# MorphIQ-Labs/VectorWave

Hardware: AMD Instinct MI355X
Metric: Msamples/sec MODWT fwd+inv db4 L=6, batch 4096×4096 fp64 @ 1/2/4/8 GPU (higher is better)
Workload: dtype f64

## Files before the change

include/vectorwave_amd.h:

```cpp
#ifndef VECTORWAVE_AMD_H
#define VECTORWAVE_AMD_H

#include <stdint.h>

#ifdef __cplusplus
extern "C" {
#endif

#define VW_API __attribute__((visibility("default")))

typedef struct vw_ctx vw_ctx;
typedef struct vw_stream vw_stream;
typedef int vw_status;

enum {
    VW_OK = 0,
    VW_ERR_NULL = 1,
    VW_ERR_EMPTY = 2,
    VW_ERR_NONFINITE = 3,
    VW_ERR_LEVEL = 4,
    VW_ERR_TOO_LARGE = 5,
    VW_ERR_BOUNDARY = 6,
    VW_ERR_ARG = 7,
    VW_ERR_DEVICE = 8,
// ... 178 lines not shown

VW_API vw_status vw_stream_create(vw_ctx *ctx, const double *lo, const double *hi, int L,
                                  int boundary, int levels, vw_stream **out);
VW_API vw_status vw_stream_destroy(vw_stream *s);
VW_API vw_status vw_stream_process_f64(vw_stream *s, const double *block, int64_t B, int64_t n,
                                       unsigned flags, double *details, double *approx);
VW_API vw_status vw_stream_flush_f64(vw_stream *s, int64_t tail_len, unsigned flags,
                                     double *details, double *approx);
VW_API int64_t vw_stream_history_length(vw_stream *s, int level);
VW_API int64_t vw_stream_batch(vw_stream *s);

typedef struct vw_graph vw_graph;
VW_API vw_status vw_capture_begin(vw_ctx *ctx);
VW_API vw_status vw_capture_end(vw_ctx *ctx, vw_graph **out);
VW_API vw_status vw_graph_launch(vw_graph *graph, int64_t count);
VW_API vw_status vw_graph_destroy(vw_graph *graph);
VW_API vw_status vw_graph_stats(vw_graph *graph, int *kernel_nodes, int *fused_pairs);

VW_API vw_status vw_modwt_roundtrip_f64(vw_ctx *ctx, const double *x, int64_t B, int64_t N, int64_t ldx,
                                        const double *lo, const double *hi, const double *rlo, const double *rhi,
                                        int L, int wavelet_id, int boundary, int J, unsigned flags, double *details,
                                        double *approx, double *y);
VW_API vw_status vw_roundtrip_occupancy(vw_ctx *ctx, int64_t N, int L, int J, unsigned flags, int *per_cu);

typedef struct vw_pipeline vw_pipeline;
VW_API vw_status vw_pipeline_create(vw_ctx *fwd_ctx, vw_ctx *inv_ctx, int elem_bytes, int sets, void *const *x,
                                    void *const *details, void *const *approx, void *const *y, int64_t B,
                                    int64_t N, const double *lo, const double *hi, int L, int wavelet_id,
                                    int boundary, int J, unsigned flags, vw_pipeline **out);
VW_API vw_status vw_pipeline_run(vw_pipeline *p, int64_t steps);
VW_API vw_status vw_pipeline_join(vw_pipeline *p);
VW_API int64_t vw_pipeline_last_set(vw_pipeline *p);
VW_API vw_status vw_pipeline_destroy(vw_pipeline *p);

VW_API vw_status vw_fill_uniform_f64(vw_ctx *ctx, double *x, int64_t count, uint64_t seed, int64_t offset);
VW_API vw_status vw_fill_uniform_f32(vw_ctx *ctx, float *x, int64_t count, uint64_t seed, int64_t offset);
VW_API vw_status vw_device_alloc(vw_ctx *ctx, int64_t bytes, void **out);
VW_API vw_status vw_device_free(vw_ctx *ctx, void *p);
VW_API vw_status vw_memcpy(vw_ctx *ctx, void *dst, const void *src, int64_t bytes, int kind );

VW_API vw_status vw_ctx_enable_timing(vw_ctx *ctx, int enable);
VW_API vw_status vw_ctx_kernel_time(vw_ctx *ctx, const char *family, double *total_ms, int64_t *launches);
VW_API vw_status vw_ctx_reset_timing(vw_ctx *ctx);
VW_API vw_status vw_ctx_kernel_spans(vw_ctx *ctx, const char *family, void *ref_event, int64_t max,
                                     double *start_ms, double *end_ms, int64_t *count);

// ... 5 lines not shown
```

vectorwave_amd/_native.py:

```python
from __future__ import annotations

import ctypes
import os
from ctypes import POINTER, c_char_p, c_double, c_float, c_int, c_int64, c_uint, c_uint64, c_void_p

_HERE = os.path.dirname(os.path.abspath(__file__))
LIB_PATH = os.environ.get("VW_LIB_PATH", os.path.join(_HERE, "libvectorwave_amd.so"))

FLAG_CORE_LEVELS = 1 << 0
FLAG_VALIDATE = 1 << 1
FLAG_FFT_SWITCH = 1 << 2
FLAG_FMA = 1 << 3
FLAG_HOST_MEMORY = 1 << 4
FLAG_SYNC = 1 << 5
FLAG_BATCH_SYM_INVERSE = 1 << 6
FLAG_BATCH_HAAR = 1 << 7
FLAG_REF_NONFINITE = 1 << 8
FLAG_TREE_SUMS = 1 << 9

PERIODIC, SYMMETRIC, ZERO_PADDING = 0, 1, 2

CWT_ZERO, CWT_REFLECT, CWT_SYMMETRIC, CWT_PERIODIC, CWT_WRAP_ZERO = 0, 1, 2, 3, 4


# ... 85 lines not shown
    "vw_stream_history_length": (c_int64, [c_void_p, c_int]),
    "vw_stream_batch": (c_int64, [c_void_p]),
    "vw_fill_uniform_f64": (c_int, [c_void_p, c_void_p, c_int64, c_uint64, c_int64]),
    "vw_fill_uniform_f32": (c_int, [c_void_p, c_void_p, c_int64, c_uint64, c_int64]),
    "vw_device_alloc": (c_int, [c_void_p, c_int64, POINTER(c_void_p)]),
    "vw_device_free": (c_int, [c_void_p, c_void_p]),
    "vw_memcpy": (c_int, [c_void_p, c_void_p, c_void_p, c_int64, c_int]),
    "vw_ctx_enable_timing": (c_int, [c_void_p, c_int]),
    "vw_ctx_kernel_time": (c_int, [c_void_p, c_char_p, POINTER(c_double), POINTER(c_int64)]),
    "vw_ctx_reset_timing": (c_int, [c_void_p]),
    "vw_ctx_kernel_spans": (c_int, [c_void_p, c_char_p, c_void_p, c_int64, POINTER(c_double), POINTER(c_double),
                                    POINTER(c_int64)]),
    "vw_median_f64": (c_int, [c_void_p, c_void_p, c_int64, c_int64, c_void_p, c_uint, c_void_p]),
    "vw_stddev_f64": (c_int, [c_void_p, c_void_p, c_int64, c_uint, c_void_p]),
    "vw_window_gather_abs_f64": (c_int, [c_void_p, c_void_p, c_void_p, c_int64, c_void_p, c_int64, c_int64]),
    "vw_capture_begin": (c_int, [c_void_p]),
    "vw_capture_end": (c_int, [c_void_p, POINTER(c_void_p)]),
    "vw_graph_launch": (c_int, [c_void_p, c_int64]),
    "vw_graph_destroy": (c_int, [c_void_p]),
    "vw_graph_stats": (c_int, [c_void_p, POINTER(c_int), POINTER(c_int)]),
    "vw_modwt_roundtrip_f64": (c_int, [c_void_p, c_void_p, c_int64, c_int64, c_int64, _dp, _dp, _dp, _dp, c_int, c_int,
                                       c_int, c_int, c_uint, c_void_p, c_void_p, c_void_p]),
    "vw_roundtrip_occupancy": (c_int, [c_void_p, c_int64, c_int, c_int, c_uint, POINTER(c_int)]),
    "vw_pipeline_create": (c_int, [c_void_p, c_void_p, c_int, c_int, c_void_p, c_void_p, c_void_p, c_void_p, c_int64,
                                   c_int64, _dp, _dp, c_int, c_int, c_int, c_int, c_uint, POINTER(c_void_p)]),
    "vw_pipeline_run": (c_int, [c_void_p, c_int64]),
    "vw_pipeline_join": (c_int, [c_void_p]),
    "vw_pipeline_last_set": (c_int64, [c_void_p]),
    "vw_pipeline_destroy": (c_int, [c_void_p]),
}

_lib = None


def load() -> ctypes.CDLL:
    global _lib
    if _lib is not None:
        return _lib
    if not os.path.exists(LIB_PATH):
        raise ImportError(
            f"vectorwave_amd native library not found at {LIB_PATH}; build it with "
            f"`python -c 'import __graft_entry__ as g; g.build()'` (make -C vectorwave_amd/csrc)")
    lib = ctypes.CDLL(LIB_PATH)
    for name, (res, args) in SIGNATURES.items():
        fn = getattr(lib, name)
        fn.restype = res
# ... 18 lines not shown
```

vectorwave_amd/csrc/vw_capi.cpp:

```cpp
#include "../../include/vectorwave_amd.h"
#include "vw_internal.h"
#include "vw_deep.h"
#include "vw_plan.h"

#include <algorithm>
#include <cmath>
#include <cstdarg>
#include <cstdio>
#include <cstring>
#include <map>
#include <mutex>
#include <set>
#include <string>
#include <thread>
#include <vector>

using namespace vw;

static thread_local std::string t_err;
static thread_local int64_t t_err_index = -1;
static thread_local int64_t t_signal_base = 0;

static vw_status fail(vw_status code, const char* fmt, ...) {
  char buf[512];
// ... 856 lines not shown
static bool capture_tail(hipStream_t st, hipGraphNode_t* node) {
  hipStreamCaptureStatus status;
  unsigned long long id = 0;
  hipGraph_t g = nullptr;
  const hipGraphNode_t* deps = nullptr;
  size_t ndeps = 0;
  if (hipStreamGetCaptureInfo_v2(st, &status, &id, &g, &deps, &ndeps) != hipSuccess) {
    (void)hipGetLastError();
    return false;
  }
  if (status != hipStreamCaptureStatusActive || ndeps != 1 || !deps) return false;
  *node = deps[0];
  return true;
}

static bool pair_forward_shape(const FwdPlan<double>& p) {
  return p.fused && p.kernel == kFwdPersist && p.args.level_ct && p.nv == 4 && p.args.taps <= kPairMaxTaps;
}

static void pair_after_forward(vw_ctx* c, const FwdCall<double>& k, const FwdPlan<double>& p, const FwdArgs<double>& a) {
  c->pair.valid = false;
  if (!c->tune.pair_fuse || !pair_forward_shape(p)) return;
  if (!c->capturing) {
    if (pair_prepare(a.taps, p.fma, p.threads, p.lds, nullptr) != hipSuccess) (void)hipGetLastError();
    return;
  }
  if (c->timing || p.ref_nf || p.validate) return;
  hipGraphNode_t node = nullptr;
  hipGraphNodeType ty;
  if (!capture_tail(c->stream, &node)) return;
  if (hipGraphNodeGetType(node, &ty) != hipSuccess || ty != hipGraphNodeTypeKernel) {
    (void)hipGetLastError();
    return;
  }
  c->pair.node = node;
  c->pair.call = k;
  c->pair.call.lo = c->pair.call.hi = nullptr;
  c->pair.plan = p;
  c->pair.args = a;
  c->pair.valid = true;
}
static void pair_after_forward(vw_ctx* c, const FwdCall<float>&, const FwdPlan<float>&, const FwdArgs<float>&) {
  c->pair.valid = false;
}

static void pair_args(const FwdArgs<double>& f, const InvCall<double>& k, const InvPlan<double>& p, PairArgs<double>* a) {
  a->f = f;
  a->y = k.y;
  double lo[kMaxTaps], hi[kMaxTaps];
  copy_bank(lo, hi, k, p.args.taps, p.args.taps_hi);
  for (int i = 0; i < kPairMaxTaps; ++i) { a->ilo[i] = lo[i]; a->ihi[i] = hi[i]; }
  for (int j = 0; j < kMaxLevels; ++j) { a->hr[j] = p.args.lv[j].hr; a->own[j] = p.args.lv[j].own; }
}

static bool try_pair_fuse(vw_ctx* c, const InvCall<double>& k, const InvPlan<double>& p) {
  const bool pending = c->pair.valid;
  c->pair.valid = false;
  if (!pending || !c->capturing || c->timing || !c->tune.pair_fuse) return false;
  hipGraphNode_t tail = nullptr;
  if (!capture_tail(c->stream, &tail) || tail != c->pair.node) return false;
  if (!pair_fusable(c->pair.call, c->pair.plan, k, p)) return false;
  const FwdPlan<double>& fp = c->pair.plan;
  PairLaunch l;
  if (!pair_launch_shape(fp.args.taps, fp.fma, fp.threads, fp.lds, k.B, c->cus, &l)) return false;
  PairArgs<double> a;
  pair_args(c->pair.args, k, p, &a);
  void* params[] = {&a};
  hipKernelNodeParams np;
  memset(&np, 0, sizeof(np));
  np.func = const_cast<void*>(l.func);
  np.gridDim = dim3(l.grid);
  np.blockDim = dim3(l.threads);
  np.sharedMemBytes = l.lds;
  np.kernelParams = params;
  if (hipGraphKernelNodeSetParams(c->pair.node, &np) != hipSuccess) {
    (void)hipGetLastError();
    return false;
  }
  ++c->fused_pairs;
  return true;
}
static bool try_pair_fuse(vw_ctx* c, const InvCall<float>&, const InvPlan<float>&) {
  c->pair.valid = false;
  return false;
}

template <typename T>
// ... 344 lines not shown
}

extern "C" vw_status vw_modwt_roundtrip_f64(vw_ctx* c, const double* x, int64_t B, int64_t N, int64_t ldx,
                                            const double* lo, const double* hi, const double* rlo, const double* rhi,
                                            int L, int wid, int boundary, int J, unsigned flags, double* details,
                                            double* approx, double* y) {
  if (c && x && details && approx && y && lo && hi && rlo && rhi && !(flags & VW_FLAG_HOST_MEMORY) && B > 0 && N > 0 &&
      ldx >= N && L >= 1 && L <= kPairMaxTaps && J >= 1 && J <= kMaxLevels && boundary == VW_PERIODIC) {
    std::lock_guard<std::recursive_mutex> g(c->mu);
    hipSetDevice(c->device);
    FwdCall<double> fk;
    fk.x = x; fk.B = B; fk.N = N; fk.ldx = ldx; fk.lo = lo; fk.hi = hi; fk.L = L; fk.boundary = boundary; fk.J = J;
    fk.flags = flags; fk.details = details; fk.approx = approx; fk.cus = c->cus;
    InvCall<double> ik;
    ik.details = details; ik.approx = approx; ik.B = B; ik.N = N; ik.lo = rlo; ik.hi = rhi; ik.L = L; ik.wid = wid;
    ik.boundary = boundary; ik.J = J; ik.flags = flags; ik.y = y; ik.cus = c->cus;
    FwdPlan<double> fp;
    InvPlan<double> ip;
    if (c->tune.pair_fuse && check_levels(N, L, J, flags) == VW_OK && capture_guard(c, flags) == VW_OK) {
      plan_forward(c->tune, fk, &fp);
      plan_inverse(c->tune, ik, &ip);
      PairLaunch l;
      if (pair_fusable(fk, fp, ik, ip) &&
          (c->capturing || pair_prepare(fp.args.taps, fp.fma, fp.threads, fp.lds, nullptr) == hipSuccess) &&
          pair_launch_shape(fp.args.taps, fp.fma, fp.threads, fp.lds, B, c->cus, &l)) {
        FwdArgs<double> f = fp.args;
        f.x = x; f.details = details; f.approx = approx;
        f.bad = c->bad;
        copy_bank(f.lo, f.hi, fk, f.taps, f.taps_hi);
        PairArgs<double> a;
        pair_args(f, ik, ip, &a);
        {
          LaunchTimer lt(c, "roundtrip");
          hipError_t e = launch_roundtrip(a, l, c->stream);
          if (e != hipSuccess) return fail(VW_ERR_DEVICE, "round-trip launch failed: %s", hipGetErrorString(e));
        }
        if (flags & VW_FLAG_SYNC) VW_HIP(hipStreamSynchronize(c->stream));
        return ok();
      }
      (void)hipGetLastError();
    }
  }
  VW_TRY(modwt_forward<double>(c, x, B, N, ldx, lo, hi, L, wid, boundary, J, flags, details, approx));
  return modwt_inverse<double>(c, details, approx, B, N, rlo, rhi, L, wid, boundary, J, ~0u, 0, flags, y);
}

extern "C" vw_status vw_roundtrip_occupancy(vw_ctx* c, int64_t N, int L, int J, unsigned flags, int* per_cu) {
  if (!c || !per_cu) return fail(VW_ERR_NULL, "null argument");
  *per_cu = 0;
  if (N <= 0 || N > (1LL << 30) || L < 1 || L > kPairMaxTaps || J < 1 || J > kMaxLevels) return ok();
  std::lock_guard<std::recursive_mutex> g(c->mu);
  if (c->capturing) return fail(VW_ERR_STATE, "occupancy queries cannot be captured");
  hipSetDevice(c->device);
  double* const aligned = reinterpret_cast<double*>(uintptr_t(4096));
  static const double taps[kPairMaxTaps] = {0};
  FwdCall<double> fk;
  fk.x = aligned; fk.details = aligned; fk.approx = aligned;
  fk.B = 4LL * c->cus; fk.N = N; fk.ldx = N; fk.lo = taps; fk.hi = taps; fk.L = L; fk.J = J;
  fk.flags = flags & VW_FLAG_FMA; fk.cus = c->cus;
  FwdPlan<double> fp;
  plan_forward(c->tune, fk, &fp);
  if (fp.error != VW_OK || !pair_forward_shape(fp)) return ok();
  if (pair_prepare(fp.args.taps, fp.fma, fp.threads, fp.lds, per_cu) != hipSuccess) {
    (void)hipGetLastError();
    *per_cu = 0;
  }
  return ok();
}

static int bank_hi(int Llo, int Lhi) { return Lhi == Llo ? 0 : Lhi; }
static vw_status bank_arg(int Lhi) {
  if (Lhi < 1 || Lhi > kMaxTaps) return fail(VW_ERR_ARG, "filter length %d unsupported (1..%d)", Lhi, kMaxTaps);
  return VW_OK;
}
extern "C" vw_status vw_modwt_forward_bi_f64(vw_ctx* c, const double* x, int64_t B, int64_t N, int64_t ldx,
                                             const double* lo, int Llo, const double* hi, int Lhi, int wid,
                                             int boundary, int J, unsigned flags, double* details, double* approx) {
  VW_TRY(bank_arg(Lhi));
  return modwt_forward<double>(c, x, B, N, ldx, lo, hi, Llo, wid, boundary, J, flags, details, approx, bank_hi(Llo, Lhi));
}
extern "C" vw_status vw_modwt_forward_bi_f32(vw_ctx* c, const float* x, int64_t B, int64_t N, int64_t ldx,
                                             const double* lo, int Llo, const double* hi, int Lhi, int wid,
                                             int boundary, int J, unsigned flags, float* details, float* approx) {
  VW_TRY(bank_arg(Lhi));
  return modwt_forward<float>(c, x, B, N, ldx, lo, hi, Llo, wid, boundary, J, flags, details, approx, bank_hi(Llo, Lhi));
}
extern "C" vw_status vw_modwt_inverse_bi_f64(vw_ctx* c, const double* details, const double* approx, int64_t B,
                                             int64_t N, const double* lo, int Llo, const double* hi, int Lhi, int wid,
                                             int boundary, int J, unsigned detail_mask, int approx_zero,
                                             unsigned flags, double* y) {
// ... 1350 lines not shown
```

vectorwave_amd/csrc/vw_internal.h:

```cpp
#pragma once
#include <hip/hip_runtime.h>
#include <atomic>
#include <cstdint>
#include "vw_taps.h"

namespace vw {

constexpr int kMaxTaps = 64;
constexpr int kMaxLevels = 24;
constexpr int kNV = 8;
constexpr int kMaxThreads = 1024;
constexpr int kLdsBytes = 160 * 1024;
constexpr int kSweepMinS = 16;
constexpr int kSweepChunk = 128;

enum HaloMode : int {
  kHaloPeriodic = 0,
  kHaloZero = 1,
  kHaloSymmetric = 2,
  kHaloFftPad = 3,
  kHaloHistory = 4
};

struct LevelDesc {
// ... 58 lines not shown
  int unrolled;
  int level_ct;
  int full;
  int plain;
  int waves;
  int db;
  int blk;
  int approx_zero;
  int rev;
  const T* thr;
  long long thr_ld;
  int soft;
  int taps;
  int taps_hi;
  int tap_lds;
  int blk_tight;
  int* nf_flag;
  T lo[kMaxTaps];
  T hi[kMaxTaps];
  LevelDesc lv[kMaxLevels];
};

constexpr int kPairMaxTaps = 8;
template <typename T>
struct PairArgs {
  FwdArgs<T> f;
  T* y;
  T ilo[kPairMaxTaps];
  T ihi[kPairMaxTaps];
  int hr[kMaxLevels];
  int own[kMaxLevels];
};

template <typename T>
struct LevelArgs {
  const T* src_a;
  long long lda;
  const T* src_d;
  const T* src_d2;
  const T* thr2;
  int use_d2;
  const T* src_d3;
  const T* thr3;
  int use_d3;
  T* out_a;
  T* out_d;
// ... 235 lines not shown
  if (lds_bytes <= 64 * 1024) return hipSuccess;
  int dev = 0;
  if (hipGetDevice(&dev) != hipSuccess || dev < 0) dev = 0;
  std::atomic<int>* f = dev < kMaxDevices ? &once->limit[dev] : nullptr;
  if (f && f->load(std::memory_order_acquire) >= lds_bytes) return hipSuccess;
  if (want < lds_bytes) want = lds_bytes;
  hipError_t e = hipFuncSetAttribute(reinterpret_cast<const void*>(k), hipFuncAttributeMaxDynamicSharedMemorySize, want);
  if (e != hipSuccess) return e;
  if (f) f->store(want, std::memory_order_release);
  return hipSuccess;
}

template <typename T>
hipError_t launch_forward_fused(const FwdArgs<T>& a, int threads, int lds_bytes, bool fma, int nv, hipStream_t st);
template <typename T>
hipError_t launch_forward_persist(const FwdArgs<T>& a, int threads, int lds_bytes, bool fma, int nv, hipStream_t st);
template <typename T>
hipError_t launch_forward_blk(const FwdArgs<T>& a, int threads, int lds_bytes, bool fma, int nv, hipStream_t st);
template <typename T>
hipError_t launch_inverse_fused(const InvArgs<T>& a, int threads, int lds_bytes, bool fma, int nv, hipStream_t st);
struct PairLaunch {
  const void* func;
  unsigned grid, threads, lds;
};
hipError_t pair_prepare(int taps, bool fma, int threads, int lds_bytes, int* per_cu);
bool pair_launch_shape(int taps, bool fma, int threads, int lds_bytes, long long B, int cus, PairLaunch* out);
hipError_t launch_roundtrip(const PairArgs<double>& a, const PairLaunch& l, hipStream_t st);
template <typename T>
hipError_t launch_forward_level(const LevelArgs<T>& a, int lds_bytes, bool fma, hipStream_t st);
template <typename T>
hipError_t launch_inverse_level(const LevelArgs<T>& a, int lds_bytes, bool fma, hipStream_t st);
template <typename T>
hipError_t launch_forward_sweep(const LevelArgs<T>& a, bool fma, hipStream_t st);
template <typename T>
hipError_t launch_inverse_sweep(const LevelArgs<T>& a, bool fma, hipStream_t st);
template <typename T>
hipError_t launch_inverse_sweepg(const LevelArgs<T>& a, int levels, int ka, int R, bool fma, hipStream_t st);
template <typename T>
hipError_t launch_forward_multi(const MultiArgs<T>& a, int lds_bytes, bool fma, hipStream_t st);

template <typename T>
hipError_t launch_inverse_multi(const MultiArgs<T>& a, int lds_bytes, bool fma, hipStream_t st);
template <typename T>
hipError_t launch_history_update(const T* level_in, long long ld_in, const T* old_hist, T* new_hist,
                                 long long B, int n, int hist_len, hipStream_t st);

hipError_t launch_level_threshold(const double* coeffs, long long level_stride, const double* sigma,
                                  const DenoiseConsts& k, long long B, int levels, double* thr, hipStream_t st);
hipError_t launch_noise_sigma(const double* coeffs, long long ld, long long B, int N, double scale_c,
// ... 32 lines not shown
```

vectorwave_amd/csrc/vw_pair.hip:

```cpp
#include "vw_device.h"

#include <algorithm>
#include <mutex>

namespace vw {

#ifndef VW_PAIR_STORE_AUX
#define VW_PAIR_STORE_AUX 16
#endif

template <typename P>
__device__ __forceinline__ const P* reread(const P* p) {
  int z = 0;
  asm volatile("" : "+s"(z));
  return p + z;
}

template <typename T, int L, bool FMA>
__global__ void __attribute__((amdgpu_flat_work_group_size(1, 512), amdgpu_waves_per_eu(4)))
k_roundtrip(const PairArgs<T> q) {
  constexpr int V = VT<T>::V;
  constexpr int NV = 4;
  const FwdArgs<T>& p = q.f;
  extern __shared__ __attribute__((aligned(16))) unsigned char smem[];
  const int N = p.N;
  const int nvec = N / V;
  const long long G = gridDim.x;
  const size_t plane = (size_t)p.B * (size_t)(unsigned)p.N;
  const unsigned slab = blockDim.x * 16u;
  long long b = blockIdx.x;
  if (b >= p.B) return;
  int cur = 0;
  dma_row<T>(reinterpret_cast<T*>(smem) + p.hlpad, p.x + b * p.ldx, nvec, p.dma_nt != 0);
  wait_vmem();
  for (;;) {
    const FwdArgs<T>& p0 = *reread(&q.f);
    T* X = reinterpret_cast<T*>(smem) + (cur ? p0.region1 : 0) + p0.hlpad;
    T* Y = reinterpret_cast<T*>(smem) + (cur ? 0 : p0.region1) + p0.hlpad;
    lds_barrier();
    fill_halo(X, p0.N, p0.lv[0].hl, p0.lv[0].hr, p0.lv[0].mode, p0.npow2, (const T*)nullptr, 0);
    const long long bn = b + G;
    const size_t row = (size_t)b * (size_t)(unsigned)N;
    const int J = p0.J;
    T acc[NV][V];
    T dlast[NV][V];
    T dreg[NV][V];
    for (int j = 1; j <= J; ++j) {
      const FwdArgs<T>& pj = *reread(&q.f);
      const LevelDesc lv = pj.lv[j - 1];
      lds_barrier();
      if (j == pj.J && bn < pj.B) dma_row<T>(Y, pj.x + bn * pj.ldx, nvec, pj.dma_nt != 0);
      T* dout = pj.details + (size_t)(j - 1) * plane + row;
      T* aout = (j == pj.J) ? pj.approx + row : nullptr;
      fwd_level<T, L, FMA, NV, false, false, true, L, VW_PAIR_STORE_AUX>(p, X, nvec, lv, dout, aout, true, 0ull, acc,
                                                                         nullptr, dlast);
      if (j < pj.J) {
        regs_to_level<T, L, NV, true>(Y, acc, nvec, pj.N, pj.lv[j], pj.npow2, (const T*)nullptr);
        T* t = X; X = Y; Y = t;
      }
    }
    const PairArgs<T>& qi = *reread(&q);
    T* const R = X - qi.f.hlpad;
    lds_barrier();
    plain_to_level<T, NV>(R, acc, slab, qi.f.N, qi.hr[qi.f.J - 1], qi.own[qi.f.J - 1]);
    for (int j = J; j >= 1; --j) {
      const PairArgs<T>& qj = *reread(&q);
      const int s = qj.f.lv[j - 1].s;
      lds_barrier();
      zero_regs<T, NV>(acc);
      plain_row<T, L, FMA, NV, 4>(R, slab, s, qj.ilo, acc);
      lds_barrier();
      if (j < qj.f.J) {
        wait_vmem();
        plain_to_level<T, NV>(R, dreg, slab, qj.f.N, qj.hr[j - 1], qj.own[j - 1]);
      } else {
        plain_to_level<T, NV>(R, dlast, slab, qj.f.N, qj.hr[j - 1], qj.own[j - 1]);
      }
      if (j > 1) {
        if (j == qj.f.J) {
          if (bn < qj.f.B) wait_vmcnt<3 * NV>();
          else wait_vmcnt<2 * NV>();
        }
        plain_load_row<T, NV>(dreg, qj.f.details + (size_t)(j - 2) * plane + row, slab);
      }
      lds_barrier();
      plain_row<T, L, FMA, NV, 4>(R, slab, s, reread(q.ihi), acc);
      if (j > 1) {
        lds_barrier();
        plain_to_level<T, NV>(R, acc, slab, qj.f.N, qj.hr[j - 2], qj.own[j - 2]);
      }
    }
    plain_store_row<T, NV>(q.y + row, acc, slab);
    if (bn >= p.B) break;
    wait_vmcnt<3 * NV>();
    cur = (cur + J) & 1;
    b = bn;
  }
}

struct PairKernel {
  static constexpr int kShapes = 16;
  const void* func = nullptr;
  LdsOnce lds;
  std::mutex mu;
  struct Shape { int threads = -1, lds = -1, per_cu = 0; } shapes[kShapes];
  int next = 0;
  int find(int threads, int lds_bytes) {
    for (const Shape& sh : shapes)
      if (sh.threads == threads && sh.lds == lds_bytes) return sh.per_cu;
    return 0;
  }
};

template <int L, bool FMA>
static PairKernel* pair_kernel_of() {
  static PairKernel k;
  k.func = reinterpret_cast<const void*>(&k_roundtrip<double, L, FMA>);
  return &k;
}

static PairKernel* pair_kernel(int taps, bool fma) {
  switch (taps) {
#define VW_CASE(n) \
    case n:        \
      if constexpr (n <= kPairMaxTaps) return fma ? pair_kernel_of<n, true>() : pair_kernel_of<n, false>(); \
      break;
    VW_TAP_LIST(VW_CASE)
#undef VW_CASE
    default: break;
  }
  return nullptr;
}

static bool lds_ready(PairKernel* k, int lds) {
  if (lds <= 64 * 1024) return true;
  int dev = 0;
  if (hipGetDevice(&dev) != hipSuccess || dev < 0 || dev >= kMaxDevices) return false;
  return k->lds.limit[dev].load(std::memory_order_acquire) >= lds;
}

hipError_t pair_prepare(int taps, bool fma, int threads, int lds, int* per_cu) {
  PairKernel* k = pair_kernel(taps, fma);
  if (!k) return hipErrorNotSupported;
  hipError_t e = set_lds(k->func, lds, &k->lds);
  if (e != hipSuccess) return e;
  std::lock_guard<std::mutex> g(k->mu);
  int n = k->find(threads, lds);
  if (!n) {
    if ((e = hipOccupancyMaxActiveBlocksPerMultiprocessor(&n, k->func, threads, lds)) != hipSuccess) return e;
    if (n < 1) return hipErrorInvalidConfiguration;
    PairKernel::Shape& sh = k->shapes[k->next];
    k->next = (k->next + 1) % PairKernel::kShapes;
    sh.threads = threads; sh.lds = lds; sh.per_cu = n;
  }
  if (per_cu) *per_cu = n;
  return hipSuccess;
}

bool pair_launch_shape(int taps, bool fma, int threads, int lds, long long B, int cus, PairLaunch* out) {
  PairKernel* k = pair_kernel(taps, fma);
  if (!k || !lds_ready(k, lds)) return false;
  int n;
  {
    std::lock_guard<std::mutex> g(k->mu);
    n = k->find(threads, lds);
  }
  if (n < 1) return false;
  out->func = k->func;
  out->grid = (unsigned)std::min<long long>(B, (long long)n * cus);
  out->threads = (unsigned)threads;
  out->lds = (unsigned)lds;
  return true;
}

hipError_t launch_roundtrip(const PairArgs<double>& a, const PairLaunch& l, hipStream_t st) {
  void* params[] = {const_cast<PairArgs<double>*>(&a)};
  return hipLaunchKernel(l.func, dim3(l.grid), dim3(l.threads), params, l.lds, st);
}

}
```

vectorwave_amd/csrc/vw_plan.cpp:

```cpp
#include "vw_plan.h"

#include <algorithm>
#include <cstdio>
#include <cstdlib>
#include <cstring>
#include <type_traits>

namespace vw {

struct TuningKey {
  const char* name;
  void (*set)(Tuning& t, const Tuning& d, int v);
};
#define VW_KEY(name, stmt) {name, [](Tuning& t, const Tuning& d, int v) { (void)d; stmt; }}
static const TuningKey kTuningTable[] = {
    VW_KEY("VW_NV", t.nv = v < 0 ? d.nv : v <= 4 ? 4 : 8),
    VW_KEY("VW_FWD_PERSIST", t.fwd_persist = v < 0 ? d.fwd_persist : v != 0),
    VW_KEY("VW_FWD_BUF", t.fwd_buf = v < 0 ? d.fwd_buf : v),
    VW_KEY("VW_FORCE_TILED", t.force_tiled = v > 0),
    VW_KEY("VW_FWD_REV", t.fwd_rev = v < 0 ? 0 : v),
    VW_KEY("VW_INV_REV", t.inv_rev = v < 0 ? 0 : v),
    VW_KEY("VW_FWD_TILE", t.fwd_tile = v < 0 ? 0 : v),
    VW_KEY("VW_MULTI", t.multi = v < 0 ? d.multi : v != 0),
    VW_KEY("VW_MULTI_DIV", t.multi_div = v <= 0 ? d.multi_div : v),
// ... 13 lines not shown
    VW_KEY("VW_DEEP", t.deep = v < 0 ? d.deep : v != 0; t.deep_inv = v < 0 ? d.deep_inv : v != 0),
    VW_KEY("VW_DEEP_INV", t.deep_inv = v < 0 ? d.deep_inv : v != 0),
    VW_KEY("VW_DEEP_LDS", t.deep_lds = v <= 0 ? d.deep_lds : v),
    VW_KEY("VW_DEEP_WAVES", t.deep_waves = v <= 0 ? d.deep_waves : v),
    VW_KEY("VW_DEEP_PF_FWD", t.deep_pf_fwd = v <= 0 ? d.deep_pf_fwd : std::min(v, 16)),
    VW_KEY("VW_DEEP_PF_INV", t.deep_pf_inv = v <= 0 ? d.deep_pf_inv : std::min(v, 16)),
    VW_KEY("VW_SWEEP2", t.sweep2 = v < 0 ? d.sweep2 : v),
    VW_KEY("VW_SWEEP2_KA", t.sweep2_ka = v == 16 ? 16 : v == 8 ? 8 : d.sweep2_ka),
    VW_KEY("VW_SWEEP2_UC", t.sweep2_uc = v >= 32 ? v : d.sweep2_uc),
    VW_KEY("VW_SWEEP2_R", t.sweep2_r = v == 32 ? 32 : 0),
    VW_KEY("VW_SWEEP2_MINB", t.sweep2_minb = v < 0 ? d.sweep2_minb : v),
    VW_KEY("VW_BLK_FWD8", t.blk_fwd8 = v < 0 ? d.blk_fwd8 : v),
    VW_KEY("VW_DMA_NT", t.dma_nt = v < 0 ? d.dma_nt : v),
    VW_KEY("VW_MULTI_NI", t.multi_ni = v < 0 ? d.multi_ni : v == 4 ? 4 : 8),
    VW_KEY("VW_MFMA", t.mfma = v < 0 ? d.mfma : v),
    VW_KEY("VW_REF_GRID", t.ref_grid = v < 0 ? d.ref_grid : v),
    VW_KEY("VW_LEVEL_CT", t.level_ct = v < 0 ? d.level_ct : v != 0),
    VW_KEY("VW_ENERGY_FUSED", t.energy_fused = v < 0 ? d.energy_fused : v),
    VW_KEY("VW_MRA_FUSED", t.mra_fused = v < 0 ? d.mra_fused : v >= 2 ? 2 : v),
    VW_KEY("VW_BI", t.bi = v < 0 ? d.bi : v & 7),
    VW_KEY("VW_BI_LISTED", t.bi_listed = v < 0 ? d.bi_listed : v != 0),
    VW_KEY("VW_INV_WAVES", t.inv_waves = v == 6 || v == 8 ? v : d.inv_waves),
    VW_KEY("VW_PAIR_FUSE", t.pair_fuse = v < 0 ? d.pair_fuse : v != 0),
};
#undef VW_KEY

bool set_tuning(Tuning& t, const char* key, int v) {
  const Tuning d;
  for (const TuningKey& k : kTuningTable)
    if (!strcmp(k.name, key)) { k.set(t, d, v); return true; }
  return false;
}

Tuning read_tuning() {
  Tuning t;
  const Tuning d;
  for (const TuningKey& k : kTuningTable) {
    const char* e = getenv(k.name);
    if (e) k.set(t, d, *e == '\0' ? 1 : atoi(e));
  }
  return t;
}


int max_levels(int64_t N, int L) {
  if (L <= 0 || N <= L) return 0;
// ... 964 lines not shown
  const unsigned off = VW_FLAG_VALIDATE | VW_FLAG_REF_NONFINITE | VW_FLAG_HOST_MEMORY;
  if ((fc.flags | ic.flags) & off) return false;
  if (fc.hist || fp.validate || fp.ref_nf || ip.ref_nf || fp.snapshot) return false;
  if (fp.kernel != kFwdPersist || !fp.args.level_ct || fp.nv != 4 || fp.args.region1 <= 0) return false;
  if (L > kPairMaxTaps || !has_unrolled_taps(L) || fp.args.taps != L || fp.args.taps_hi != L) return false;
  const InvArgs<T>& ia = ip.args;
  if (ip.threads != fp.threads || ip.nv != 4 || ia.taps != L || ia.taps_hi != L) return false;
  if (!ia.plain && !(ip.kernel == kInvDb && plain_class(ic, ip, ip.nv))) return false;
  for (int j = 0; j < J; ++j)
    if (ia.lv[j].s != fp.args.lv[j].s || N + ia.lv[j].hr > fp.args.region1) return false;
  if (fp.lds < 2 * fp.args.region1 * (int)sizeof(T)) return false;
  const size_t row = (size_t)N * sizeof(T), plane = (size_t)B * row;
  const size_t x_bytes = ((size_t)(B - 1) * (size_t)fc.ldx + (size_t)N) * sizeof(T);
  if (ranges_overlap(ic.y, plane, fc.x, x_bytes) || ranges_overlap(ic.y, plane, fc.details, (size_t)J * plane) ||
      ranges_overlap(ic.y, plane, fc.approx, plane))
    return false;
  return true;
}
template bool pair_fusable<float>(const FwdCall<float>&, const FwdPlan<float>&, const InvCall<float>&,
                                  const InvPlan<float>&);
template bool pair_fusable<double>(const FwdCall<double>&, const FwdPlan<double>&, const InvCall<double>&,
                                   const InvPlan<double>&);

template void plan_forward<float>(const Tuning&, const FwdCall<float>&, FwdPlan<float>*);
template void plan_forward<double>(const Tuning&, const FwdCall<double>&, FwdPlan<double>*);
template void plan_inverse<float>(const Tuning&, const InvCall<float>&, InvPlan<float>*);
template void plan_inverse<double>(const Tuning&, const InvCall<double>&, InvPlan<double>*);

}
```

vectorwave_amd/csrc/vw_plan.h:

```cpp
#pragma once
#include "../../include/vectorwave_amd.h"
#include "vw_internal.h"
#include "vw_deep.h"

#include <vector>

namespace vw {

struct Tuning {
  int nv = 4;
  bool fwd_persist = true;
  int fwd_buf = 0;
  bool force_tiled = false;
  int fwd_rev = 0, inv_rev = 0;
  int dma_nt = -1;
  int fwd_tile = 0;
  bool multi = true;
  int multi_div = 4;
  int multi_tile = 0;
  int inv_buf = 0;
  int inv_tile = 0;
  int multi_rblk = 1;
  int multi_pf = 1;
  int multi_pad = 1;
// ... 5 lines not shown
  int blk = 10;
  bool deep = true;
  bool deep_inv = false;
  int deep_lds = 80;
  int deep_waves = 4;
  int deep_pf_fwd = 1;
  int deep_pf_inv = 1;
  int fwd_nv = 0;
  int inv_nv = 0;
  int sweep2 = 3;
  int sweep2_ka = 8;
  int sweep2_uc = 2048;
  int sweep2_r = 0;
  int sweep2_minb = 64;
  int blk_fwd8 = 1;
  int ref_grid = 0;
  int level_ct = 1;
  int mfma = 0;
  int energy_fused = 1;
  int bi = 3;
  int inv_waves = 6;
  int mra_fused = 1;
  int pair_fuse = 1;
  int bi_listed = 1;
};

bool set_tuning(Tuning& t, const char* key, int v);
Tuning read_tuning();

int max_levels(int64_t N, int L);
int64_t upsampled_length(int L, int level);
int ref_mode(int boundary);

template <typename T>
struct FwdCall {
  const T* x = nullptr;
  int64_t B = 0, N = 0, ldx = 0;
  const double* lo = nullptr;
  const double* hi = nullptr;
  int L = 0, boundary = VW_PERIODIC, J = 1;
  unsigned flags = 0;
  T* details = nullptr;
  T* approx = nullptr;
  bool single_level = false;
  int mode_override = -1;
  T* const* hist = nullptr;
// ... 131 lines not shown
```

vectorwave_amd/engine.py:

```python
from __future__ import annotations

import ctypes
import threading
from ctypes import byref, c_double, c_int64, c_void_p
from typing import Optional, Sequence, Tuple

import numpy as np

from . import _native as nat
from .errors import InvalidArgumentException, raise_for_status

try:
    import torch
except Exception:
    torch = None


def _is_device_tensor(a) -> bool:
    return torch is not None and isinstance(a, torch.Tensor) and a.is_cuda


def _one_length(lo, hi, what: str) -> int:
    if len(lo) != len(hi):
        raise InvalidArgumentException(f"{what} takes one filter length, got {len(lo)} low-pass and {len(hi)} "
# ... 173 lines not shown

    def roundtrip(self, x, lo, hi, rlo, rhi, wavelet_id: int, boundary: int, levels: int, flags: int):
        xa, dev, xp, _ = self._prep(x, np.float64)
        one = xa.ndim == 1
        B, N = (1, xa.shape[0]) if one else xa.shape
        det = self._empty(xa, dev, (levels, N) if one else (levels, B, N))
        app = self._empty(xa, dev, xa.shape)
        y = self._empty(xa, dev, xa.shape)
        L = _one_length(lo, hi, "roundtrip")
        if _one_length(rlo, rhi, "roundtrip") != L:
            raise InvalidArgumentException("roundtrip takes one filter length for both pairs")
        _check(self.lib.vw_modwt_roundtrip_f64(self.ctx, xp, B, N, N, nat.taps_array(lo), nat.taps_array(hi),
                                               nat.taps_array(rlo), nat.taps_array(rhi), L, wavelet_id, boundary,
                                               levels, self._flags(flags, dev), self._ptr(det, dev),
                                               self._ptr(app, dev), self._ptr(y, dev)))
        return det, app, y

    def roundtrip_occupancy(self, N: int, L: int, levels: int, flags: int = 0) -> int:
        from ctypes import c_int
        n = c_int()
        _check(self.lib.vw_roundtrip_occupancy(self.ctx, int(N), int(L), int(levels), int(flags), byref(n)))
        return n.value

    def forward1(self, x, lo, hi, boundary: int, flags: int):
        xa, dev, xp, f32 = self._prep(x, np.float64)
        one = xa.ndim == 1
        B, N = (1, xa.shape[0]) if one else xa.shape
        app = self._empty(xa, dev, xa.shape)
        det = self._empty(xa, dev, xa.shape)
        if len(lo) != len(hi):
            _check(self.lib.vw_modwt1_forward_bi_f64(self.ctx, xp, B, N, N, nat.taps_array(lo), len(lo),
                                                     nat.taps_array(hi), len(hi), boundary, self._flags(flags, dev),
                                                     self._ptr(app, dev), self._ptr(det, dev)))
            return app, det
        _check(self.lib.vw_modwt1_forward_f64(self.ctx, xp, B, N, N, nat.taps_array(lo), nat.taps_array(hi), len(lo),
                                              boundary, self._flags(flags, dev), self._ptr(app, dev),
                                              self._ptr(det, dev)))
        return app, det

    def inverse1(self, approx, detail, lo, hi, boundary: int, flags: int):
        aa, dev, ap, _ = self._prep(approx, np.float64)
        da, _, dp, _ = self._prep(detail, np.float64)
        one = aa.ndim == 1
        B, N = (1, aa.shape[0]) if one else aa.shape
        y = self._empty(aa, dev, aa.shape)
        if len(lo) != len(hi):
# ... 231 lines not shown
```

Baseline: 52740.

## Keep last forward detail planes in registers for fused roundtrip inverse

Adds templated roundtrip kernel variants that hold the last one or two forward detail levels in registers, so the inverse pass can skip reloading them from global memory. By default the variant is picked automatically: the highest keep count whose occupancy per CU matches the keep-0 kernel. Also adds an API and env knob to query or force the variant. The extra registers can reduce occupancy, and the auto selection guards against that.

```diff
diff --git a/include/vectorwave_amd.h b/include/vectorwave_amd.h
--- a/include/vectorwave_amd.h
+++ b/include/vectorwave_amd.h
@@ -224,6 +224,7 @@
                                         int L, int wavelet_id, int boundary, int J, unsigned flags, double *details,
                                         double *approx, double *y);
 VW_API vw_status vw_roundtrip_occupancy(vw_ctx *ctx, int64_t N, int L, int J, unsigned flags, int *per_cu);
+VW_API vw_status vw_roundtrip_variant(vw_ctx *ctx, int64_t N, int L, int J, unsigned flags, int *keep, int *per_cu);
 
 typedef struct vw_pipeline vw_pipeline;
 VW_API vw_status vw_pipeline_create(vw_ctx *fwd_ctx, vw_ctx *inv_ctx, int elem_bytes, int sets, void *const *x,
diff --git a/vectorwave_amd/_native.py b/vectorwave_amd/_native.py
--- a/vectorwave_amd/_native.py
+++ b/vectorwave_amd/_native.py
@@ -131,6 +131,7 @@
     "vw_modwt_roundtrip_f64": (c_int, [c_void_p, c_void_p, c_int64, c_int64, c_int64, _dp, _dp, _dp, _dp, c_int, c_int,
                                        c_int, c_int, c_uint, c_void_p, c_void_p, c_void_p]),
     "vw_roundtrip_occupancy": (c_int, [c_void_p, c_int64, c_int, c_int, c_uint, POINTER(c_int)]),
+    "vw_roundtrip_variant": (c_int, [c_void_p, c_int64, c_int, c_int, c_uint, POINTER(c_int), POINTER(c_int)]),
     "vw_pipeline_create": (c_int, [c_void_p, c_void_p, c_int, c_int, c_void_p, c_void_p, c_void_p, c_void_p, c_int64,
                                    c_int64, _dp, _dp, c_int, c_int, c_int, c_int, c_uint, POINTER(c_void_p)]),
     "vw_pipeline_run": (c_int, [c_void_p, c_int64]),
diff --git a/vectorwave_amd/csrc/vw_capi.cpp b/vectorwave_amd/csrc/vw_capi.cpp
--- a/vectorwave_amd/csrc/vw_capi.cpp
+++ b/vectorwave_amd/csrc/vw_capi.cpp
@@ -902,7 +902,7 @@
   c->pair.valid = false;
   if (!c->tune.pair_fuse || !pair_forward_shape(p)) return;
   if (!c->capturing) {
-    if (pair_prepare(a.taps, p.fma, p.threads, p.lds, nullptr) != hipSuccess) (void)hipGetLastError();
+    if (pair_prepare(a.taps, p.fma, p.threads, p.lds, c->tune.pair_keep, nullptr, nullptr) != hipSuccess) (void)hipGetLastError();
     return;
   }
   if (c->timing || p.ref_nf || p.validate) return;
@@ -942,7 +942,7 @@
   if (!pair_fusable(c->pair.call, c->pair.plan, k, p)) return false;
   const FwdPlan<double>& fp = c->pair.plan;
   PairLaunch l;
-  if (!pair_launch_shape(fp.args.taps, fp.fma, fp.threads, fp.lds, k.B, c->cus, &l)) return false;
+  if (!pair_launch_shape(fp.args.taps, fp.fma, fp.threads, fp.lds, c->tune.pair_keep, k.B, c->cus, &l)) return false;
   PairArgs<double> a;
   pair_args(c->pair.args, k, p, &a);
   void* params[] = {&a};
@@ -1333,8 +1333,9 @@
       plan_inverse(c->tune, ik, &ip);
       PairLaunch l;
       if (pair_fusable(fk, fp, ik, ip) &&
-          (c->capturing || pair_prepare(fp.args.taps, fp.fma, fp.threads, fp.lds, nullptr) == hipSuccess) &&
-          pair_launch_shape(fp.args.taps, fp.fma, fp.threads, fp.lds, B, c->cus, &l)) {
+          (c->capturing ||
+           pair_prepare(fp.args.taps, fp.fma, fp.threads, fp.lds, c->tune.pair_keep, nullptr, nullptr) == hipSuccess) &&
+          pair_launch_shape(fp.args.taps, fp.fma, fp.threads, fp.lds, c->tune.pair_keep, B, c->cus, &l)) {
         FwdArgs<double> f = fp.args;
         f.x = x; f.details = details; f.approx = approx;
         f.bad = c->bad;
@@ -1356,9 +1357,8 @@
   return modwt_inverse<double>(c, details, approx, B, N, rlo, rhi, L, wid, boundary, J, ~0u, 0, flags, y);
 }
 
-extern "C" vw_status vw_roundtrip_occupancy(vw_ctx* c, int64_t N, int L, int J, unsigned flags, int* per_cu) {
-  if (!c || !per_cu) return fail(VW_ERR_NULL, "null argument");
-  *per_cu = 0;
+static vw_status roundtrip_variant(vw_ctx* c, int64_t N, int L, int J, unsigned flags, int* keep, int* per_cu) {
+  *keep = *per_cu = 0;
   if (N <= 0 || N > (1LL << 30) || L < 1 || L > kPairMaxTaps || J < 1 || J > kMaxLevels) return ok();
   std::lock_guard<std::recursive_mutex> g(c->mu);
   if (c->capturing) return fail(VW_ERR_STATE, "occupancy queries cannot be captured");
@@ -1372,11 +1372,22 @@
   FwdPlan<double> fp;
   plan_forward(c->tune, fk, &fp);
   if (fp.error != VW_OK || !pair_forward_shape(fp)) return ok();
-  if (pair_prepare(fp.args.taps, fp.fma, fp.threads, fp.lds, per_cu) != hipSuccess) {
+  if (pair_prepare(fp.args.taps, fp.fma, fp.threads, fp.lds, c->tune.pair_keep, per_cu, keep) != hipSuccess) {
     (void)hipGetLastError();
-    *per_cu = 0;
-  }
-  return ok();
+    *keep = *per_cu = 0;
+  }
+  return ok();
+}
+
+extern "C" vw_status vw_roundtrip_occupancy(vw_ctx* c, int64_t N, int L, int J, unsigned flags, int* per_cu) {
+  if (!c || !per_cu) return fail(VW_ERR_NULL, "null argument");
+  int keep;
+  return roundtrip_variant(c, N, L, J, flags, &keep, per_cu);
+}
+
+extern "C" vw_status vw_roundtrip_variant(vw_ctx* c, int64_t N, int L, int J, unsigned flags, int* keep, int* per_cu) {
+  if (!c || !keep || !per_cu) return fail(VW_ERR_NULL, "null argument");
+  return roundtrip_variant(c, N, L, J, flags, keep, per_cu);
 }
 
 static int bank_hi(int Llo, int Lhi) { return Lhi == Llo ? 0 : Lhi; }
diff --git a/vectorwave_amd/csrc/vw_internal.h b/vectorwave_amd/csrc/vw_internal.h
--- a/vectorwave_amd/csrc/vw_internal.h
+++ b/vectorwave_amd/csrc/vw_internal.h
@@ -104,6 +104,9 @@
 };
 
 constexpr int kPairMaxTaps = 8;
+constexpr int kPairMaxKeep = 2;
+constexpr int kPairAutoKeep = 2;
+int pair_keep_variant(int requested, const int (&per_cu)[kPairMaxKeep + 1]);
 template <typename T>
 struct PairArgs {
   FwdArgs<T> f;
@@ -385,9 +388,10 @@
 struct PairLaunch {
   const void* func;
   unsigned grid, threads, lds;
-};
-hipError_t pair_prepare(int taps, bool fma, int threads, int lds_bytes, int* per_cu);
-bool pair_launch_shape(int taps, bool fma, int threads, int lds_bytes, long long B, int cus, PairLaunch* out);
+  int keep, per_cu;
+};
+hipError_t pair_prepare(int taps, bool fma, int threads, int lds_bytes, int keep, int* per_cu, int* variant);
+bool pair_launch_shape(int taps, bool fma, int threads, int lds_bytes, int keep, long long B, int cus, PairLaunch* out);
 hipError_t launch_roundtrip(const PairArgs<double>& a, const PairLaunch& l, hipStream_t st);
 template <typename T>
 hipError_t launch_forward_level(const LevelArgs<T>& a, int lds_bytes, bool fma, hipStream_t st);
diff --git a/vectorwave_amd/csrc/vw_pair.hip b/vectorwave_amd/csrc/vw_pair.hip
--- a/vectorwave_amd/csrc/vw_pair.hip
+++ b/vectorwave_amd/csrc/vw_pair.hip
@@ -16,86 +16,26 @@
   return p + z;
 }
 
+template <typename T, int NV>
+__device__ __forceinline__ void copy_regs(T (&to)[NV][VT<T>::V], const T (&from)[NV][VT<T>::V]) {
+#pragma unroll
+  for (int k = 0; k < NV; ++k)
+#pragma unroll
+    for (int e = 0; e < VT<T>::V; ++e) to[k][e] = from[k][e];
+}
+
 template <typename T, int L, bool FMA>
 __global__ void __attribute__((amdgpu_flat_work_group_size(1, 512), amdgpu_waves_per_eu(4)))
 k_roundtrip(const PairArgs<T> q) {
-  constexpr int V = VT<T>::V;
-  constexpr int NV = 4;
-  const FwdArgs<T>& p = q.f;
-  extern __shared__ __attribute__((aligned(16))) unsigned char smem[];
-  const int N = p.N;
-  const int nvec = N / V;
-  const long long G = gridDim.x;
-  const size_t plane = (size_t)p.B * (size_t)(unsigned)p.N;
-  const unsigned slab = blockDim.x * 16u;
-  long long b = blockIdx.x;
-  if (b >= p.B) return;
-  int cur = 0;
-  dma_row<T>(reinterpret_cast<T*>(smem) + p.hlpad, p.x + b * p.ldx, nvec, p.dma_nt != 0);
-  wait_vmem();
-  for (;;) {
-    const FwdArgs<T>& p0 = *reread(&q.f);
-    T* X = reinterpret_cast<T*>(smem) + (cur ? p0.region1 : 0) + p0.hlpad;
-    T* Y = reinterpret_cast<T*>(smem) + (cur ? 0 : p0.region1) + p0.hlpad;
-    lds_barrier();
-    fill_halo(X, p0.N, p0.lv[0].hl, p0.lv[0].hr, p0.lv[0].mode, p0.npow2, (const T*)nullptr, 0);
-    const long long bn = b + G;
-    const size_t row = (size_t)b * (size_t)(unsigned)N;
-    const int J = p0.J;
-    T acc[NV][V];
-    T dlast[NV][V];
-    T dreg[NV][V];
-    for (int j = 1; j <= J; ++j) {
-      const FwdArgs<T>& pj = *reread(&q.f);
-      const LevelDesc lv = pj.lv[j - 1];
-      lds_barrier();
-      if (j == pj.J && bn < pj.B) dma_row<T>(Y, pj.x + bn * pj.ldx, nvec, pj.dma_nt != 0);
-      T* dout = pj.details + (size_t)(j - 1) * plane + row;
-      T* aout = (j == pj.J) ? pj.approx + row : nullptr;
-      fwd_level<T, L, FMA, NV, false, false, true, L, VW_PAIR_STORE_AUX>(p, X, nvec, lv, dout, aout, true, 0ull, acc,
-                                                                         nullptr, dlast);
-      if (j < pj.J) {
-        regs_to_level<T, L, NV, true>(Y, acc, nvec, pj.N, pj.lv[j], pj.npow2, (const T*)nullptr);
-        T* t = X; X = Y; Y = t;
-      }
-    }
-    const PairArgs<T>& qi = *reread(&q);
-    T* const R = X - qi.f.hlpad;
-    lds_barrier();
-    plain_to_level<T, NV>(R, acc, slab, qi.f.N, qi.hr[qi.f.J - 1], qi.own[qi.f.J - 1]);
-    for (int j = J; j >= 1; --j) {
-      const PairArgs<T>& qj = *reread(&q);
-      const int s = qj.f.lv[j - 1].s;
-      lds_barrier();
-      zero_regs<T, NV>(acc);
-      plain_row<T, L, FMA, NV, 4>(R, slab, s, qj.ilo, acc);
-      lds_barrier();
-      if (j < qj.f.J) {
-        wait_vmem();
-        plain_to_level<T, NV>(R, dreg, slab, qj.f.N, qj.hr[j - 1], qj.own[j - 1]);
-      } else {
-        plain_to_level<T, NV>(R, dlast, slab, qj.f.N, qj.hr[j - 1], qj.own[j - 1]);
-      }
-      if (j > 1) {
-        if (j == qj.f.J) {
-          if (bn < qj.f.B) wait_vmcnt<3 * NV>();
-          else wait_vmcnt<2 * NV>();
-        }
-        plain_load_row<T, NV>(dreg, qj.f.details + (size_t)(j - 2) * plane + row, slab);
-      }
-      lds_barrier();
-      plain_row<T, L, FMA, NV, 4>(R, slab, s, reread(q.ihi), acc);
-      if (j > 1) {
-        lds_barrier();
-        plain_to_level<T, NV>(R, acc, slab, qj.f.N, qj.hr[j - 2], qj.own[j - 2]);
-      }
-    }
-    plain_store_row<T, NV>(q.y + row, acc, slab);
-    if (bn >= p.B) break;
-    wait_vmcnt<3 * NV>();
-    cur = (cur + J) & 1;
-    b = bn;
-  }
+  constexpr int KEEP = 0;
+#include "vw_pair_rows.inc"
+}
+
+template <typename T, int L, bool FMA, int KEEP>
+__global__ void __attribute__((amdgpu_flat_work_group_size(1, 512), amdgpu_waves_per_eu(4)))
+k_rtrip_keep(const PairArgs<T> q) {
+  static_assert(KEEP >= 1 && KEEP <= kPairMaxKeep, "KEEP = 0 is k_roundtrip; a third kept plane spills");
+#include "vw_pair_rows.inc"
 }
 
 struct PairKernel {
@@ -112,18 +52,26 @@
   }
 };
 
-template <int L, bool FMA>
+template <int L, bool FMA, int KEEP>
 static PairKernel* pair_kernel_of() {
   static PairKernel k;
-  k.func = reinterpret_cast<const void*>(&k_roundtrip<double, L, FMA>);
+  if constexpr (KEEP == 0) k.func = reinterpret_cast<const void*>(&k_roundtrip<double, L, FMA>);
+  else k.func = reinterpret_cast<const void*>(&k_rtrip_keep<double, L, FMA, KEEP>);
   return &k;
 }
 
-static PairKernel* pair_kernel(int taps, bool fma) {
+template <int L, bool FMA>
+static PairKernel* pair_kernel_keep(int keep) {
+  static_assert(kPairMaxKeep == 2, "one case per variant");
+  return keep == 0 ? pair_kernel_of<L, FMA, 0>() : keep == 1 ? pair_kernel_of<L, FMA, 1>() : pair_kernel_of<L, FMA, 2>();
+}
+
+static PairKernel* pair_kernel(int taps, bool fma, int keep) {
+  if (keep < 0 || keep > kPairMaxKeep) return nullptr;
   switch (taps) {
 #define VW_CASE(n) \
     case n:        \
-      if constexpr (n <= kPairMaxTaps) return fma ? pair_kernel_of<n, true>() : pair_kernel_of<n, false>(); \
+      if constexpr (n <= kPairMaxTaps) return fma ? pair_kernel_keep<n, true>(keep) : pair_kernel_keep<n, false>(keep); \
       break;
     VW_TAP_LIST(VW_CASE)
 #undef VW_CASE
@@ -139,9 +87,7 @@
   return k->lds.limit[dev].load(std::memory_order_acquire) >= lds;
 }
 
-hipError_t pair_prepare(int taps, bool fma, int threads, int lds, int* per_cu) {
-  PairKernel* k = pair_kernel(taps, fma);
-  if (!k) return hipErrorNotSupported;
+static hipError_t prepare_variant(PairKernel* k, int threads, int lds, int* per_cu) {
   hipError_t e = set_lds(k->func, lds, &k->lds);
   if (e != hipSuccess) return e;
   std::lock_guard<std::mutex> g(k->mu);
@@ -153,23 +99,40 @@
     k->next = (k->next + 1) % PairKernel::kShapes;
     sh.threads = threads; sh.lds = lds; sh.per_cu = n;
   }
-  if (per_cu) *per_cu = n;
+  *per_cu = n;
   return hipSuccess;
 }
 
-bool pair_launch_shape(int taps, bool fma, int threads, int lds, long long B, int cus, PairLaunch* out) {
-  PairKernel* k = pair_kernel(taps, fma);
-  if (!k || !lds_ready(k, lds)) return false;
-  int n;
-  {
+hipError_t pair_prepare(int taps, bool fma, int threads, int lds, int keep, int* per_cu, int* variant) {
+  int n[kPairMaxKeep + 1];
+  for (int v = 0; v <= kPairMaxKeep; ++v) {
+    PairKernel* k = pair_kernel(taps, fma, v);
+    if (!k) return hipErrorNotSupported;
+    hipError_t e = prepare_variant(k, threads, lds, &n[v]);
+    if (e != hipSuccess) return e;
+  }
+  const int v = pair_keep_variant(keep, n);
+  if (per_cu) *per_cu = n[v];
+  if (variant) *variant = v;
+  return hipSuccess;
+}
+
+bool pair_launch_shape(int taps, bool fma, int threads, int lds, int keep, long long B, int cus, PairLaunch* out) {
+  int n[kPairMaxKeep + 1];
+  PairKernel* ks[kPairMaxKeep + 1];
+  for (int v = 0; v <= kPairMaxKeep; ++v) {
+    PairKernel* k = ks[v] = pair_kernel(taps, fma, v);
+    if (!k || !lds_ready(k, lds)) return false;
     std::lock_guard<std::mutex> g(k->mu);
-    n = k->find(threads, lds);
+    if ((n[v] = k->find(threads, lds)) < 1) return false;
   }
-  if (n < 1) return false;
-  out->func = k->func;
-  out->grid = (unsigned)std::min<long long>(B, (long long)n * cus);
+  const int v = pair_keep_variant(keep, n);
+  out->func = ks[v]->func;
+  out->grid = (unsigned)std::min<long long>(B, (long long)n[v] * cus);
   out->threads = (unsigned)threads;
   out->lds = (unsigned)lds;
+  out->keep = v;
+  out->per_cu = n[v];
   return true;
 }
 
diff --git a/vectorwave_amd/csrc/vw_pair_rows.inc b/vectorwave_amd/csrc/vw_pair_rows.inc
--- /dev/null
+++ b/vectorwave_amd/csrc/vw_pair_rows.inc
@@ -0,0 +1,87 @@
+  constexpr int V = VT<T>::V;
+  constexpr int NV = 4;
+  const FwdArgs<T>& p = q.f;
+  extern __shared__ __attribute__((aligned(16))) unsigned char smem[];
+  const int N = p.N;
+  const int nvec = N / V;
+  const long long G = gridDim.x;
+  const size_t plane = (size_t)p.B * (size_t)(unsigned)p.N;
+  const unsigned slab = blockDim.x * 16u;
+  long long b = blockIdx.x;
+  if (b >= p.B) return;
+  int cur = 0;
+  dma_row<T>(reinterpret_cast<T*>(smem) + p.hlpad, p.x + b * p.ldx, nvec, p.dma_nt != 0);
+  wait_vmem();
+  for (;;) {
+    const FwdArgs<T>& p0 = *reread(&q.f);
+    T* X = reinterpret_cast<T*>(smem) + (cur ? p0.region1 : 0) + p0.hlpad;
+    T* Y = reinterpret_cast<T*>(smem) + (cur ? 0 : p0.region1) + p0.hlpad;
+    lds_barrier();
+    fill_halo(X, p0.N, p0.lv[0].hl, p0.lv[0].hr, p0.lv[0].mode, p0.npow2, (const T*)nullptr, 0);
+    const long long bn = b + G;
+    const size_t row = (size_t)b * (size_t)(unsigned)N;
+    const int J = p0.J;
+    T acc[NV][V];
+    T dlast[NV][V];
+    T dreg[NV][V];
+    T dk[KEEP > 0 ? KEEP : 1][NV][V];
+    for (int j = 1; j <= J; ++j) {
+      const FwdArgs<T>& pj = *reread(&q.f);
+      const LevelDesc lv = pj.lv[j - 1];
+      lds_barrier();
+      if (j == pj.J && bn < pj.B) dma_row<T>(Y, pj.x + bn * pj.ldx, nvec, pj.dma_nt != 0);
+      T* dout = pj.details + (size_t)(j - 1) * plane + row;
+      T* aout = (j == pj.J) ? pj.approx + row : nullptr;
+      if constexpr (KEEP > 1) copy_regs<T, NV>(dk[1], dk[0]);
+      if constexpr (KEEP > 0) copy_regs<T, NV>(dk[0], dlast);
+      fwd_level<T, L, FMA, NV, false, false, true, L, VW_PAIR_STORE_AUX>(p, X, nvec, lv, dout, aout, true, 0ull, acc,
+                                                                         nullptr, dlast);
+      if (j < pj.J) {
+        regs_to_level<T, L, NV, true>(Y, acc, nvec, pj.N, pj.lv[j], pj.npow2, (const T*)nullptr);
+        T* t = X; X = Y; Y = t;
+      }
+    }
+    const PairArgs<T>& qi = *reread(&q);
+    T* const R = X - qi.f.hlpad;
+    lds_barrier();
+    plain_to_level<T, NV>(R, acc, slab, qi.f.N, qi.hr[qi.f.J - 1], qi.own[qi.f.J - 1]);
+    for (int j = J; j >= 1; --j) {
+      const PairArgs<T>& qj = *reread(&q);
+      const int s = qj.f.lv[j - 1].s;
+      lds_barrier();
+      zero_regs<T, NV>(acc);
+      plain_row<T, L, FMA, NV, 4>(R, slab, s, qj.ilo, acc);
+      lds_barrier();
+      if (j + KEEP < qj.f.J) {
+        wait_vmem();
+        plain_to_level<T, NV>(R, dreg, slab, qj.f.N, qj.hr[j - 1], qj.own[j - 1]);
+      } else {
+        bool shifted = false;
+        if constexpr (KEEP > 0) {
+          if (j + 1 == qj.f.J) { shifted = true; plain_to_level<T, NV>(R, dk[0], slab, qj.f.N, qj.hr[j - 1], qj.own[j - 1]); }
+        }
+        if constexpr (KEEP > 1) {
+          if (j + 2 == qj.f.J) { shifted = true; plain_to_level<T, NV>(R, dk[1], slab, qj.f.N, qj.hr[j - 1], qj.own[j - 1]); }
+        }
+        if (!shifted) plain_to_level<T, NV>(R, dlast, slab, qj.f.N, qj.hr[j - 1], qj.own[j - 1]);
+      }
+      if (j > 1 && (KEEP == 0 || j + KEEP <= qj.f.J)) {
+        if (j + KEEP == qj.f.J) {
+          if (bn < qj.f.B) wait_vmcnt<3 * NV>();
+          else wait_vmcnt<2 * NV>();
+        }
+        plain_load_row<T, NV>(dreg, qj.f.details + (size_t)(j - 2) * plane + row, slab);
+      }
+      lds_barrier();
+      plain_row<T, L, FMA, NV, 4>(R, slab, s, reread(q.ihi), acc);
+      if (j > 1) {
+        lds_barrier();
+        plain_to_level<T, NV>(R, acc, slab, qj.f.N, qj.hr[j - 2], qj.own[j - 2]);
+      }
+    }
+    plain_store_row<T, NV>(q.y + row, acc, slab);
+    if (bn >= p.B) break;
+    wait_vmcnt<3 * NV>();
+    cur = (cur + J) & 1;
+    b = bn;
+  }
diff --git a/vectorwave_amd/csrc/vw_plan.cpp b/vectorwave_amd/csrc/vw_plan.cpp
--- a/vectorwave_amd/csrc/vw_plan.cpp
+++ b/vectorwave_amd/csrc/vw_plan.cpp
@@ -59,6 +59,7 @@
     VW_KEY("VW_BI_LISTED", t.bi_listed = v < 0 ? d.bi_listed : v != 0),
     VW_KEY("VW_INV_WAVES", t.inv_waves = v == 6 || v == 8 ? v : d.inv_waves),
     VW_KEY("VW_PAIR_FUSE", t.pair_fuse = v < 0 ? d.pair_fuse : v != 0),
+    VW_KEY("VW_PAIR_KEEP", t.pair_keep = v < 0 ? d.pair_keep : std::min(v, kPairMaxKeep)),
 };
 #undef VW_KEY
 
@@ -1069,6 +1070,13 @@
 template bool pair_fusable<double>(const FwdCall<double>&, const FwdPlan<double>&, const InvCall<double>&,
                                    const InvPlan<double>&);
 
+int pair_keep_variant(int requested, const int (&per_cu)[kPairMaxKeep + 1]) {
+  if (requested >= 0) return std::min(requested, kPairMaxKeep);
+  int v = kPairAutoKeep;
+  while (v > 0 && per_cu[v] < per_cu[0]) --v;
+  return v;
+}
+
 template void plan_forward<float>(const Tuning&, const FwdCall<float>&, FwdPlan<float>*);
 template void plan_forward<double>(const Tuning&, const FwdCall<double>&, FwdPlan<double>*);
 template void plan_inverse<float>(const Tuning&, const InvCall<float>&, InvPlan<float>*);
diff --git a/vectorwave_amd/csrc/vw_plan.h b/vectorwave_amd/csrc/vw_plan.h
--- a/vectorwave_amd/csrc/vw_plan.h
+++ b/vectorwave_amd/csrc/vw_plan.h
@@ -51,6 +51,7 @@
   int inv_waves = 6;
   int mra_fused = 1;
   int pair_fuse = 1;
+  int pair_keep = -1;
   int bi_listed = 1;
 };
 
diff --git a/vectorwave_amd/engine.py b/vectorwave_amd/engine.py
--- a/vectorwave_amd/engine.py
+++ b/vectorwave_amd/engine.py
@@ -219,6 +219,12 @@
         _check(self.lib.vw_roundtrip_occupancy(self.ctx, int(N), int(L), int(levels), int(flags), byref(n)))
         return n.value
 
+    def roundtrip_variant(self, N: int, L: int, levels: int, flags: int = 0):
+        from ctypes import c_int
+        keep, n = c_int(), c_int()
+        _check(self.lib.vw_roundtrip_variant(self.ctx, int(N), int(L), int(levels), int(flags), byref(keep), byref(n)))
+        return keep.value, n.value
+
     def forward1(self, x, lo, hi, boundary: int, flags: int):
         xa, dev, xp, f32 = self._prep(x, np.float64)
         one = xa.ndim == 1
```

Result: faster. 53910, median of 6 (+2.2%).
